# fanzhongyi/ExploreMultiModal

Hardware: AMD Instinct MI355X
Metric: image-text pairs/sec fwd+bwd, VLMo-Base, 1/2/4/8 MI355X; % bf16 MFMA roofline (higher is better)
Workload: dtype bf16

## Files before the change

### exploremultimodal_amd/csrc/attention.hip

```cpp
#include "common.h"
#include "vlmo_hip.h"

namespace {

struct AttnArgs {
    const bf16* qkv;
    const bf16* ctx;
    const bf16* dctx;
    bf16* out;
    float* lse;
    float* qvsum;
    const int32_t* seg;
    const int32_t* keymask;
    int lse_stride, heads, d;
    float scale, scale_log2e;
    uint32_t drop_thresh, drop_cmp;
    float inv_keep;
    uint64_t seed;
    int bh0;
};

#define LOG2E 1.4426950408889634f
#define LN2 0.6931471805599453f

// ... 314 lines not shown
        if (kt + 1 < nq) {
            if (kt + 2 < nq) S0 = s_tile(kt + 2);
            __builtin_amdgcn_sched_barrier(0);
            consume(S1, kt + 1);
            __builtin_amdgcn_sched_barrier(0);
        }
    }
    const float l_run = l2[0] + l2[1];
    const float l_tot = l_run + other_half(l_run);
    if (qi < N) {
        const float inv = a.inv_keep / l_tot;
        bf16* op = a.out + (size_t)qrow * a.d + hd * 64 + 4 * h;
#pragma unroll
        for (int dt = 0; dt < 2; ++dt)
#pragma unroll
            for (int g4 = 0; g4 < 4; ++g4) {
                bf16x4 o = {(bf16)(O[dt][4 * g4 + 0] * inv), (bf16)(O[dt][4 * g4 + 1] * inv),
                            (bf16)(O[dt][4 * g4 + 2] * inv), (bf16)(O[dt][4 * g4 + 3] * inv)};
                *(bf16x4*)(op + dt * 32 + 8 * g4) = o;
            }
        if (h == 0 && a.lse) a.lse[(size_t)bh * a.lse_stride + qi] = (m_run * c2 + log2f(l_tot)) * LN2;
    }
}

__device__ __forceinline__ float half_wave_total(float v) {
    float s_ = v + dpp_mov<0x111, 0xf, 0xf>(v);
    s_ += dpp_mov<0x112, 0xf, 0xf>(v);
    s_ += dpp_mov<0x113, 0xf, 0xf>(v);
    s_ += dpp_mov<0x114, 0xf, 0xe>(s_);
    s_ += dpp_mov<0x118, 0xf, 0xc>(s_);
    s_ += dpp_mov<0x142, 0xa, 0xf>(s_);
    return s_;
}
__device__ __forceinline__ void colsum_tiles(const f32x16* t, float w, float scale, float* acc, int lane) {
    const int h = lane >> 5;
#pragma unroll
    for (int dt = 0; dt < 2; ++dt)
#pragma unroll
        for (int r = 0; r < 16; ++r) {
            const float v = half_wave_total(t[dt][r] * w);
            if ((lane & 31) == 31) atomicAdd(acc + dt * 32 + (r & 3) + 8 * (r >> 2) + 4 * h, v * scale);
        }
}

__global__ __launch_bounds__(512, 2) void attn_bwd_kernel(const AttnArgs a, const int NPAD) {
    const int IMG = NPAD * 128;
    extern __shared__ __attribute__((aligned(16))) char smem[];
    char* Qimg = smem;
    char* Kimg = smem + IMG;
    char* Vimg = smem + 2 * IMG;
    char* Dimg = smem + 3 * IMG;
    float* kbias = (float*)(smem + 4 * IMG);
    float* lseq = kbias + NPAD;
    float* delta = lseq + NPAD;
    int* rowidx = (int*)(delta + NPAD);
    int* next_item = rowidx + NPAD;
    float* csum = (float*)(next_item + 4);

    const int lane = threadIdx.x & 63;
    const int wave = __builtin_amdgcn_readfirstlane(threadIdx.x >> 6);
    const int bh = blockIdx.x, sidx = bh / a.heads, hd = bh % a.heads;
    const int ld = 3 * a.d;
    int N;
    setup_rows(a.seg, sidx, a.keymask, NPAD, rowidx, kbias, N);
    if (threadIdx.x == 0) *next_item = 0;
    if (threadIdx.x < 128) csum[threadIdx.x] = 0.f;
    __syncthreads();
    const int nq = (N + 31) >> 5;
    stage_image<8>(a.qkv, ld, hd * 64, rowidx, Qimg, nq * 4, wave, lane);
    stage_image<8>(a.qkv, ld, a.d + hd * 64, rowidx, Kimg, nq * 4, wave, lane);
    stage_image<8>(a.qkv, ld, 2 * a.d + hd * 64, rowidx, Vimg, nq * 4, wave, lane);
    stage_image<8>(a.dctx, a.d, hd * 64, rowidx, Dimg, nq * 4, wave, lane);
    const float keep_prob = 1.f / a.inv_keep;
    for (int i = threadIdx.x; i < NPAD; i += 512) {
        float dl = 0.f, lq = INFINITY;
        if (i < N) {
            const size_t o = (size_t)rowidx[i] * a.d + hd * 64;
#pragma unroll
            for (int c = 0; c < 8; ++c) {
                const bf16x8 x = *(const bf16x8*)(a.ctx + o + 8 * c);
                const bf16x8 y = *(const bf16x8*)(a.dctx + o + 8 * c);
#pragma unroll
                for (int j = 0; j < 8; ++j) dl += (float)x[j] * (float)y[j];
            }
            lq = a.lse[(size_t)bh * a.lse_stride + i] * LOG2E;
        }
        delta[i] = dl * keep_prob;
        lseq[i] = lq;
    }
    asm volatile("s_waitcnt vmcnt(0)" ::: "memory");
    __syncthreads();

    const int l31 = lane & 31, h = lane >> 5;
    const uint32_t akey = att_key(a.seed, bh + a.bh0);
    const float out_scale = a.scale * a.inv_keep;

    f32x16 cs[2] = {zero16(), zero16()};
    int cs_kind = -1;
    for (;;) {
    int item = 0;
    if (lane == 0) item = atomicAdd(next_item, 1);
    item = __builtin_amdgcn_readfirstlane(item);
    if (a.qvsum) {
        const int kind = item >= 2 * nq ? -1 : (item >= nq ? 0 : 1);
        if (cs_kind >= 0 && kind != cs_kind) {
            colsum_tiles(cs, 1.f, cs_kind == 0 ? out_scale : a.inv_keep, csum + 64 * cs_kind, lane);
            cs[0] = zero16(), cs[1] = zero16();
        }
        cs_kind = kind;
    }
    if (item >= 2 * nq) break;
    if (item >= nq) {
        const int qt = item - nq;
        const int qi = qt * 32 + l31;
        bf16x8 qf[4], df[4];
#pragma unroll
        for (int s = 0; s < 4; ++s) {
            qf[s] = row_frag(Qimg, qt * 32, s, lane);
            df[s] = row_frag(Dimg, qt * 32, s, lane);
        }
        const float lq = lseq[qi], dl = delta[qi];
        const uint32_t rq = ((uint32_t)qi * 512u + 4u * h) * ATT_G + akey;
        f32x16 dQ[2] = {zero16(), zero16()};
        for (int kt = 0; kt < nq; ++kt) {
            {
                f32x16 S = zero16(), dP = zero16();
#pragma unroll
                for (int s = 0; s < 4; ++s) {
                    S = Elem<bf16>::mfma(row_frag(Kimg, kt * 32, s, lane), qf[s], S);
                    dP = Elem<bf16>::mfma(row_frag(Vimg, kt * 32, s, lane), df[s], dP);
                }
                const uint32_t rk = rq + (uint32_t)(kt * 32) * ATT_G;
#pragma unroll
                for (int g4 = 0; g4 < 4; ++g4) {
                    const f32x4 kb = *(const f32x4*)(kbias + kt * 32 + 8 * g4 + 4 * h);
#pragma unroll
                    for (int e = 0; e < 4; ++e) {
                        const int i = 4 * g4 + e;
                        const float p = __builtin_amdgcn_exp2f(S[i] * a.scale_log2e + (kb[e] - lq));
                        bool keep = true;
                        if (a.drop_thresh) keep = att_mix(rk + (uint32_t)(8 * g4 + e) * ATT_G) >= a.drop_cmp;
                        const float dp = keep ? dP[i] : 0.f;
                        S[i] = p * (dp - dl);
                    }
                }
#pragma unroll
                for (int s2 = 0; s2 < 2; ++s2) {
                    bf16x8 sf;
#pragma unroll
                    for (int j = 0; j < 8; ++j) sf[j] = (bf16)S[8 * s2 + j];
#pragma unroll
                    for (int dt = 0; dt < 2; ++dt)
                        dQ[dt] = Elem<bf16>::mfma(tr_frag(Kimg, kt * 32 + 16 * s2, dt * 32, lane), sf, dQ[dt]);
                }
            }
        }
        if (a.qvsum) {
            const float wq = qi < N ? 1.f : 0.f;
#pragma unroll
            for (int dt = 0; dt < 2; ++dt)
#pragma unroll
                for (int r = 0; r < 16; ++r) cs[dt][r] = fmaf(dQ[dt][r], wq, cs[dt][r]);
        }
        if (qi < N) {
            bf16* op = a.out + (size_t)rowidx[qi] * ld + hd * 64 + 4 * h;
#pragma unroll
            for (int dt = 0; dt < 2; ++dt)
#pragma unroll
                for (int g4 = 0; g4 < 4; ++g4) {
                    bf16x4 o = {(bf16)(dQ[dt][4 * g4 + 0] * out_scale), (bf16)(dQ[dt][4 * g4 + 1] * out_scale),
                                (bf16)(dQ[dt][4 * g4 + 2] * out_scale), (bf16)(dQ[dt][4 * g4 + 3] * out_scale)};
                    *(bf16x4*)(op + dt * 32 + 8 * g4) = o;
                }
        }
    }

    else {
        const int kt = item;
        const int ki = kt * 32 + l31;
        bf16x8 kf[4], vf[4];
#pragma unroll
        for (int s = 0; s < 4; ++s) {
            kf[s] = row_frag(Kimg, kt * 32, s, lane);
            vf[s] = row_frag(Vimg, kt * 32, s, lane);
        }
        const float kb = kbias[ki];
        const uint32_t rl = (uint32_t)ki * ATT_G + akey + (uint32_t)(4 * h) * ATT_G512;
        f32x16 dK[2] = {zero16(), zero16()}, dV[2] = {zero16(), zero16()};
        for (int qt = 0; qt < nq; ++qt) {
            {
                f32x16 S = zero16(), dP = zero16();
#pragma unroll
                for (int s = 0; s < 4; ++s) {
                    S = Elem<bf16>::mfma(row_frag(Qimg, qt * 32, s, lane), kf[s], S);
                    dP = Elem<bf16>::mfma(row_frag(Dimg, qt * 32, s, lane), vf[s], dP);
                }
                f32x16 Pd;
                const uint32_t rqt = rl + (uint32_t)(qt * 32) * ATT_G512;
#pragma unroll
                for (int g4 = 0; g4 < 4; ++g4) {
                    const int q0 = qt * 32 + 8 * g4 + 4 * h;
                    const f32x4 lq = *(const f32x4*)(lseq + q0);
                    const f32x4 dl = *(const f32x4*)(delta + q0);
#pragma unroll
                    for (int e = 0; e < 4; ++e) {
                        const int i = 4 * g4 + e;
                        const float p = __builtin_amdgcn_exp2f(S[i] * a.scale_log2e + (kb - lq[e]));
                        bool keep = true;
                        if (a.drop_thresh) keep = att_mix(rqt + (uint32_t)(8 * g4 + e) * ATT_G512) >= a.drop_cmp;
                        Pd[i] = keep ? p : 0.f;
                        S[i] = p * ((keep ? dP[i] : 0.f) - dl[e]);
                    }
                }
#pragma unroll
                for (int s2 = 0; s2 < 2; ++s2) {
                    bf16x8 pf, sf;
#pragma unroll
                    for (int j = 0; j < 8; ++j) {
                        pf[j] = (bf16)Pd[8 * s2 + j];
                        sf[j] = (bf16)S[8 * s2 + j];
                    }
#pragma unroll
                    for (int dt = 0; dt < 2; ++dt) {
                        dV[dt] = Elem<bf16>::mfma(tr_frag(Dimg, qt * 32 + 16 * s2, dt * 32, lane), pf, dV[dt]);
                        dK[dt] = Elem<bf16>::mfma(tr_frag(Qimg, qt * 32 + 16 * s2, dt * 32, lane), sf, dK[dt]);
                    }
                }
            }
        }
        if (a.qvsum) {
            const float wk = ki < N ? 1.f : 0.f;
#pragma unroll
            for (int dt = 0; dt < 2; ++dt)
#pragma unroll
                for (int r = 0; r < 16; ++r) cs[dt][r] = fmaf(dV[dt][r], wk, cs[dt][r]);
        }
        if (ki < N) {
            bf16* op = a.out + (size_t)rowidx[ki] * ld + hd * 64 + 4 * h;
#pragma unroll
            for (int dt = 0; dt < 2; ++dt)
#pragma unroll
                for (int g4 = 0; g4 < 4; ++g4) {
                    bf16x4 ok = {(bf16)(dK[dt][4 * g4 + 0] * out_scale), (bf16)(dK[dt][4 * g4 + 1] * out_scale),
                                 (bf16)(dK[dt][4 * g4 + 2] * out_scale), (bf16)(dK[dt][4 * g4 + 3] * out_scale)};
                    bf16x4 ov = {(bf16)(dV[dt][4 * g4 + 0] * a.inv_keep), (bf16)(dV[dt][4 * g4 + 1] * a.inv_keep),
                                 (bf16)(dV[dt][4 * g4 + 2] * a.inv_keep), (bf16)(dV[dt][4 * g4 + 3] * a.inv_keep)};
                    *(bf16x4*)(op + a.d + dt * 32 + 8 * g4) = ok;
                    *(bf16x4*)(op + 2 * a.d + dt * 32 + 8 * g4) = ov;
                }
        }
    }
    }
    if (a.qvsum) {
        __syncthreads();
        if (threadIdx.x < 128)
            a.qvsum[(size_t)sidx * 2 * a.d + (threadIdx.x >> 6) * a.d + hd * 64 + (threadIdx.x & 63)] = csum[threadIdx.x];
    }
}

__device__ __forceinline__ int slot_off(int k, int q) {
    return k * 64 + ((((q >> 2) ^ (k >> 1)) & 7) << 3) + (q & 3) * 2;
}
__global__ __launch_bounds__(512) void attn_bwd1_kernel(const AttnArgs a, const int NPAD) {
    constexpr bool KF_REG = false;
    const int IMG = NPAD * 128;
    extern __shared__ __attribute__((aligned(16))) char smem[];
    char* Qimg = smem;
    char* Dimg = smem + IMG;
    char* Kimg = smem + 2 * IMG;
    const int nt = NPAD >> 5;
    char* slots = smem + 3 * IMG;
    float* kbias = (float*)(slots + 2 * nt * 2048);
    float* nlq = kbias + NPAD;
    float* ndl = nlq + NPAD;
    float* csum = ndl + NPAD;


    const int lane = threadIdx.x & 63;
    const int w = __builtin_amdgcn_readfirstlane(threadIdx.x >> 6);
    const int nw = blockDim.x >> 6;
    const int bh = blockIdx.x, sidx = bh / a.heads, hd = bh % a.heads;
    const int ld = 3 * a.d;
    const int rowA = a.seg[4 * sidx + 0], lenA = a.seg[4 * sidx + 1], rowB = a.seg[4 * sidx + 2], lenB = a.seg[4 * sidx + 3];
    const int N = lenA + lenB;
    auto rowof = [&](int tok) {
        tok = min(tok, N - 1);
        return tok < lenA ? rowA + tok : rowB + (tok - lenA);
    };
    const int nq = (N + 31) >> 5;
    for (int ii = w; ii < nq * 4; ii += nw) {
        const int chhi = lane >> 5, rowlo = (lane >> 2) & 7, pc = lane & 3;
        const int row = ii * 8 + rowlo;
        const int ch = chhi * 4 + (pc ^ ((row >> 2) & 3));
        const size_t r = (size_t)rowof(row);
        glds16(a.qkv + r * ld + hd * 64 + ch * 8, Qimg + ii * 1024);
        glds16(a.qkv + r * ld + a.d + hd * 64 + ch * 8, Kimg + ii * 1024);
        glds16(a.dctx + r * a.d + hd * 64 + ch * 8, Dimg + ii * 1024);
    }
    const int l31 = lane & 31, h = lane >> 5;
    const bool active = w < nq;
    const int ki = w * 32 + l31;
    const int krow = rowof(ki);
    bf16x8 kf[4], vf[4];
    if (active) {
        const bf16* kp = a.qkv + (size_t)krow * ld + a.d + hd * 64 + 8 * h;
#pragma unroll
        for (int s = 0; s < 4; ++s) {
            if (KF_REG) kf[s] = *(const bf16x8*)(kp + 16 * s);
            vf[s] = *(const bf16x8*)(kp + a.d + 16 * s);
        }
    }
    for (int i = threadIdx.x; i < 128; i += blockDim.x) csum[i] = 0.f;
    const float keep_prob = 1.f / a.inv_keep;
    const float inv_scale = 1.f / a.scale;
    for (int i = threadIdx.x; i < NPAD; i += blockDim.x) {
        float dl = 0.f, lq = INFINITY;
        const int row = rowof(i);
        const bool ok = (i < N) && (!a.keymask || a.keymask[row] != 0);
        if (i < N) {
            const size_t o = (size_t)row * a.d + hd * 64;
            bf16x8 x[8], y[8];
#pragma unroll
            for (int c = 0; c < 8; ++c) {
                x[c] = *(const bf16x8*)(a.ctx + o + 8 * c);
                y[c] = *(const bf16x8*)(a.dctx + o + 8 * c);
            }
            lq = a.lse[(size_t)bh * a.lse_stride + i];
#pragma unroll
            for (int c = 0; c < 8; ++c)
#pragma unroll
                for (int j = 0; j < 8; ++j) dl += (float)x[c][j] * (float)y[c][j];
        }
        kbias[i] = ok ? 0.f : -INFINITY;
        ndl[i] = -dl * keep_prob;
        nlq[i] = -lq * inv_scale;
    }
    asm volatile("s_waitcnt vmcnt(0)" ::: "memory");
    __syncthreads();

    const uint32_t akey = att_key(a.seed, bh + a.bh0);
    const float out_scale = a.scale * a.inv_keep;
    const float c_l2 = a.scale_log2e;
    const float kb = kbias[min(ki, NPAD - 1)];
    const uint32_t rl = (uint32_t)ki * ATT_G + akey + (uint32_t)(4 * h) * ATT_G512;
    f32x16 dK[2] = {zero16(), zero16()}, dV[2] = {zero16(), zero16()}, dQ[2] = {zero16(), zero16()};

    const int xq = (l31 >> 2) & 3;
    const int rf0 = 1024 * (l31 >> 3) + 64 * (l31 & 7) + 16 * (h ^ xq);
    const int rf1 = 1024 * (l31 >> 3) + 64 * (l31 & 7) + 16 * ((2 + h) ^ xq);
    const int tg = (lane >> 4) & 1, tq = (lane >> 2) & 3, tp = lane & 3;
    const int trl = 64 * (4 * h + tq) + 16 * ((2 * tg + (tp >> 1)) ^ h) + 8 * (tp & 1);
    const int trh = 1024 + 64 * (4 * h + tq) + 16 * ((2 * tg + (tp >> 1)) ^ ((2 + h) & 3)) + 8 * (tp & 1);
    auto rfrag = [&](const char* img_rb, int s) -> bf16x8 {
        return *(const bf16x8*)(img_rb + 512 * (s >> 1) + ((s & 1) ? rf1 : rf0));
    };
    auto tfrag = [&](const char* img_rb, int dt) -> bf16x8 {
        const bf16x4 lo = lds_tr4<bf16>(img_rb + 512 * dt + trl);
        const bf16x4 hi = lds_tr4<bf16>(img_rb + 512 * dt + trh);
        return bf16x8{lo[0], lo[1], lo[2], lo[3], hi[0], hi[1], hi[2], hi[3]};
    };
    const int sw0 = slot_off(l31, 4 * h), sw1 = slot_off(l31, 8 + 4 * h);
    const int srl = slot_off(4 * h + tq, 16 * tg + 4 * tp), srh = slot_off(8 + 4 * h + tq, 16 * tg + 4 * tp);
    auto sfrag = [&](const char* slot, int s2) -> bf16x8 {
        const bf16x4 lo = lds_tr4<bf16>(slot + 1024 * s2 + srl);
        const bf16x4 hi = lds_tr4<bf16>(slot + 1024 * s2 + srh);
        return bf16x8{lo[0], lo[1], lo[2], lo[3], hi[0], hi[1], hi[2], hi[3]};
    };

    bf16x8 qa[4], da[4], pf[2], sf[2];
    f32x16 S, dP;
    auto fetch_a = [&](int qt_) {
#pragma unroll
        for (int s = 0; s < 4; ++s) {
            qa[s] = rfrag(Qimg + qt_ * 4096, s);
            da[s] = rfrag(Dimg + qt_ * 4096, s);
        }
    };
    auto qtile = [&](int t_) {
        int q_ = w + t_;
        return q_ >= nq ? q_ - nq : q_;
    };
    auto stage_sdp = [&](int qt) {
        dP = zero16();
#pragma unroll
        for (int g4 = 0; g4 < 4; ++g4) {
            const f32x4 l4 = *(const f32x4*)(nlq + qt * 32 + 8 * g4 + 4 * h);
#pragma unroll
            for (int e = 0; e < 4; ++e) S[4 * g4 + e] = l4[e];
        }
#pragma unroll
        for (int s = 0; s < 4; ++s) {
            const bf16x8 kfs = KF_REG ? kf[s] : rfrag(Kimg + w * 4096, s);
            S = Elem<bf16>::mfma(qa[s], kfs, S);
            dP = Elem<bf16>::mfma(da[s], vf[s], dP);
        }
        __builtin_amdgcn_sched_barrier(0);
    };
    auto stage_valu_dvdk = [&](int qt, int t) {
        bf16x8 dtr[2], qtr[2];
#pragma unroll
        for (int dt = 0; dt < 2; ++dt) {
            dtr[dt] = tfrag(Dimg + qt * 4096, dt);
            qtr[dt] = tfrag(Qimg + qt * 4096, dt);
        }
        __builtin_amdgcn_sched_barrier(0);
        if (a.drop_thresh) {
            const uint32_t rqt = rl + (uint32_t)(qt * 32) * ATT_G512;
#pragma unroll
            for (int g4 = 0; g4 < 4; ++g4) {
                const f32x4 nd = *(const f32x4*)(ndl + qt * 32 + 8 * g4 + 4 * h);
#pragma unroll
                for (int e = 0; e < 4; ++e) {
                    const int i = 4 * g4 + e;
                    const float p = __builtin_amdgcn_exp2f(fmaf(S[i], c_l2, kb));
                    const bool keep = att_mix(rqt + (uint32_t)(8 * g4 + e) * ATT_G512) >= a.drop_cmp;
                    const float pd = keep ? p : 0.f;
                    pf[i >> 3][i & 7] = (bf16)pd;
                    sf[i >> 3][i & 7] = (bf16)fmaf(pd, dP[i], p * nd[e]);
                }
            }
        } else {
#pragma unroll
            for (int g4 = 0; g4 < 4; ++g4) {
                const f32x4 nd = *(const f32x4*)(ndl + qt * 32 + 8 * g4 + 4 * h);
#pragma unroll
                for (int e = 0; e < 4; ++e) {
                    const int i = 4 * g4 + e;
                    const float p = __builtin_amdgcn_exp2f(fmaf(S[i], c_l2, kb));
                    pf[i >> 3][i & 7] = (bf16)p;
                    sf[i >> 3][i & 7] = (bf16)(p * (dP[i] + nd[e]));
                }
            }
        }
        char* myslot = slots + ((t & 1) * nt + w) * 2048;
#pragma unroll
        for (int s2 = 0; s2 < 2; ++s2) {
            *(bf16x4*)(myslot + (sw0 ^ (32 * s2))) = bf16x4{sf[s2][0], sf[s2][1], sf[s2][2], sf[s2][3]};
            *(bf16x4*)(myslot + (sw1 ^ (32 * s2))) = bf16x4{sf[s2][4], sf[s2][5], sf[s2][6], sf[s2][7]};
        }
        __builtin_amdgcn_sched_barrier(0);
        bf16x8 dtr1[2], qtr1[2];
#pragma unroll
        for (int dt = 0; dt < 2; ++dt) {
            dtr1[dt] = tfrag(Dimg + qt * 4096 + 2048, dt);
            qtr1[dt] = tfrag(Qimg + qt * 4096 + 2048, dt);
        }
#pragma unroll
        for (int dt = 0; dt < 2; ++dt) {
            dV[dt] = Elem<bf16>::mfma(dtr[dt], pf[0], dV[dt]);
            dK[dt] = Elem<bf16>::mfma(qtr[dt], sf[0], dK[dt]);
        }
#pragma unroll
        for (int dt = 0; dt < 2; ++dt) {
            dV[dt] = Elem<bf16>::mfma(dtr1[dt], pf[1], dV[dt]);
            dK[dt] = Elem<bf16>::mfma(qtr1[dt], sf[1], dK[dt]);
        }
        __builtin_amdgcn_sched_barrier(0);
    };
    auto stage_dq = [&](int t, int next_q) {
        int wp = w - t;
        if (wp < 0) wp += nq;
        const char* slot = slots + ((t & 1) * nt + wp) * 2048;
        bf16x8 ktr[2][2], sb[2];
#pragma unroll
        for (int s2 = 0; s2 < 2; ++s2) {
            sb[s2] = sfrag(slot, s2);
#pragma unroll
            for (int dt = 0; dt < 2; ++dt) ktr[s2][dt] = tfrag(Kimg + wp * 4096 + 2048 * s2, dt);
        }
        if (next_q >= 0) fetch_a(next_q);
        __builtin_amdgcn_sched_barrier(0);
#pragma unroll
        for (int s2 = 0; s2 < 2; ++s2)
#pragma unroll
            for (int dt = 0; dt < 2; ++dt) dQ[dt] = Elem<bf16>::mfma(ktr[s2][dt], sb[s2], dQ[dt]);
        __builtin_amdgcn_sched_barrier(0);
    };
    if (w >= 4) __builtin_amdgcn_s_setprio(1);
    if (!active) {
        for (int t = 0; t < nq; ++t) __syncthreads();
    } else if (w < 4) {
        fetch_a(w);
        for (int t = 0; t < nq; ++t) {
            const int qt = qtile(t);
            stage_sdp(qt);
            stage_valu_dvdk(qt, t);
            __syncthreads();
            stage_dq(t, t + 1 < nq ? qtile(t + 1) : -1);
        }
    } else {
        fetch_a(w);
        stage_sdp(w);
        for (int t = 0; t < nq; ++t) {
            stage_valu_dvdk(qtile(t), t);
            if (t > 0) stage_dq(t - 1, -1);
            if (t + 1 < nq) {
                fetch_a(qtile(t + 1));
                stage_sdp(qtile(t + 1));
            }
            __syncthreads();
        }
        stage_dq(nq - 1, -1);
    }
    if (active && ki < N) {
        bf16* op = a.out + (size_t)krow * ld + hd * 64 + 4 * h;
#pragma unroll
        for (int dt = 0; dt < 2; ++dt)
#pragma unroll
            for (int g4 = 0; g4 < 4; ++g4) {
                bf16x4 oq = {(bf16)(dQ[dt][4 * g4 + 0] * out_scale), (bf16)(dQ[dt][4 * g4 + 1] * out_scale),
                             (bf16)(dQ[dt][4 * g4 + 2] * out_scale), (bf16)(dQ[dt][4 * g4 + 3] * out_scale)};
                bf16x4 ok = {(bf16)(dK[dt][4 * g4 + 0] * out_scale), (bf16)(dK[dt][4 * g4 + 1] * out_scale),
                             (bf16)(dK[dt][4 * g4 + 2] * out_scale), (bf16)(dK[dt][4 * g4 + 3] * out_scale)};
                bf16x4 ov = {(bf16)(dV[dt][4 * g4 + 0] * a.inv_keep), (bf16)(dV[dt][4 * g4 + 1] * a.inv_keep),
                             (bf16)(dV[dt][4 * g4 + 2] * a.inv_keep), (bf16)(dV[dt][4 * g4 + 3] * a.inv_keep)};
                *(bf16x4*)(op + dt * 32 + 8 * g4) = oq;
                *(bf16x4*)(op + a.d + dt * 32 + 8 * g4) = ok;
                *(bf16x4*)(op + 2 * a.d + dt * 32 + 8 * g4) = ov;
            }
    }
    if (a.qvsum) {
        if (active) {
            const float wt = ki < N ? 1.f : 0.f;
            colsum_tiles(dQ, wt, out_scale, csum, lane);
            colsum_tiles(dV, wt, a.inv_keep, csum + 64, lane);
        }
        __syncthreads();
        for (int i = threadIdx.x; i < 128; i += blockDim.x) {
            float* dst = a.qvsum + (size_t)sidx * 2 * a.d + (i >> 6) * a.d + hd * 64 + (i & 63);
            *dst = csum[i];
        }
    }
}

#define ATT_LW 8
#define ATT_LCH 4
#define ATT_LBUF (ATT_LCH * 4096)
#define ATT_LMAX 1024
#define ATT_LDS_FWD (4 * ATT_LBUF + ATT_LMAX * 4)
#define ATT_LDS_BWD (4 * ATT_LBUF + 3 * ATT_LMAX * 4 + ATT_LW * 64 * 4)

__device__ __forceinline__ uint32_t att_stride(int N) { return N > 512 ? 1024u : 512u; }

struct SeqRows {
    int rowA, lenA, rowB, N;
    __device__ __forceinline__ SeqRows(const int32_t* seg, int sidx)
        : rowA(seg[4 * sidx + 0]), lenA(seg[4 * sidx + 1]), rowB(seg[4 * sidx + 2]), N(seg[4 * sidx + 1] + seg[4 * sidx + 3]) {}
    __device__ __forceinline__ int row(int tok) const {
        tok = min(tok, N - 1);
        return tok < lenA ? rowA + tok : rowB + (tok - lenA);
    }
};

__device__ __forceinline__ void stage_chunk(const bf16* pa, int lda, const bf16* pb, int ldb, const SeqRows& sr, int t0,
                                            int nt, char* ia, char* ib, int w, int lane) {
// ... 748 lines not shown
int& lds_limit_set(int which) {
    static int lim[4][64];
    static bool init = false;
    if (!init) {
        for (auto& r : lim)
            for (int& v : r) v = 65536;
        init = true;
    }
    int dev = 0;
    (void)hipGetDevice(&dev);
    return lim[which][dev & 63];
}

int launch_fwd(const AttnArgs& a, int nt, int nblocks, hipStream_t st) {
    const int LDS = nt * 32 * 256 + nt * 32 * 8;
    int& max_set = lds_limit_set(0);
    if (LDS > max_set) {
        (void)hipFuncSetAttribute((const void*)attn_fwd_kernel, hipFuncAttributeMaxDynamicSharedMemorySize, LDS);
        max_set = LDS;
    }
    hipLaunchKernelGGL(attn_fwd_kernel, dim3(nblocks), dim3(256), LDS, st, a, nt * 32);
    return 0;
}
int launch_fwd1(const AttnArgs& a, int nt, int nblocks, hipStream_t st) {
    const int LDS = nt * 32 * 256 + nt * 32 * 4;
    int& max_set = lds_limit_set(3);
    if (LDS > max_set) {
        (void)hipFuncSetAttribute((const void*)attn_fwd1_kernel, hipFuncAttributeMaxDynamicSharedMemorySize, LDS);
        max_set = LDS;
    }
    hipLaunchKernelGGL(attn_fwd1_kernel, dim3(nblocks), dim3(nt * 64), LDS, st, a, nt * 32);
    return 0;
}
int launch_bwd(const AttnArgs& a, int nt, int nblocks, hipStream_t st) {
    const int LDS = nt * 32 * 512 + nt * 32 * 16 + 32 + 512;
    int& max_set = lds_limit_set(1);
    if (LDS > max_set) {
        (void)hipFuncSetAttribute((const void*)attn_bwd_kernel, hipFuncAttributeMaxDynamicSharedMemorySize, LDS);
        max_set = LDS;
    }
    hipLaunchKernelGGL(attn_bwd_kernel, dim3(nblocks), dim3(512), LDS, st, a, nt * 32);
    return 0;
}

int launch_bwd1(const AttnArgs& a, int nt, int nblocks, hipStream_t st) {
    const int LDS = nt * 32 * 384 + 2 * nt * 2048 + nt * 32 * 12 + 512;
    int& max_set = lds_limit_set(2);
    if (LDS > max_set) {
        (void)hipFuncSetAttribute((const void*)attn_bwd1_kernel, hipFuncAttributeMaxDynamicSharedMemorySize, LDS);
        max_set = LDS;
    }
    hipLaunchKernelGGL(attn_bwd1_kernel, dim3(nblocks), dim3(nt * 64), LDS, st, a, nt * 32);
    return 0;
}

int check_common(const char* fn, const void* qkv, const int32_t* seg, int num_seq, int heads, int d, int max_len,
                 int cap) {
    VLMO_CHECK_ARG(qkv && seg, "%s: null pointer", fn);
    VLMO_CHECK_ARG(num_seq > 0 && heads > 0, "%s: empty problem", fn);
    VLMO_CHECK_ARG(d == heads * 64, "%s: head_dim must be 64 (d=%d, heads=%d)", fn, d, heads);
    VLMO_CHECK_ARG(max_len > 0 && max_len <= cap, "%s: sequence length %d exceeds this build's limit %d", fn, max_len, cap);
    return 0;
}

}

extern "C" int vlmo_attn_fwd(const void* qkv, const int32_t* seg, int num_seq, const int32_t* keymask, void* ctx,
                             float* lse, int lse_stride, int heads, int d, int max_len, float scale,
                             uint32_t drop_thresh, float inv_keep, uint64_t seed, int mask_seq0, hipStream_t stream) {
    if (int rc = check_common("vlmo_attn_fwd", qkv, seg, num_seq, heads, d, max_len, 1024)) return rc;
    VLMO_CHECK_ARG(ctx, "vlmo_attn_fwd: null ctx");
    VLMO_CHECK_ARG(!lse || lse_stride >= max_len, "vlmo_attn_fwd: lse_stride too small");
    AttnArgs a{};
    a.qkv = (const bf16*)qkv;
    a.out = (bf16*)ctx;
    a.lse = lse;
    a.seg = seg;
    a.keymask = keymask;
    a.lse_stride = lse_stride;
    a.heads = heads;
    a.d = d;
    a.scale = scale;
    a.scale_log2e = scale * LOG2E;
    a.drop_thresh = drop_thresh;
    a.drop_cmp = drop_thresh >= 65536u ? 0xFFFFFFFFu : drop_thresh << 16;
// ... 14 lines not shown

extern "C" int vlmo_attn_bwd(const void* qkv, const void* ctx, const void* dctx, const float* lse, int lse_stride,
                             const int32_t* seg, int num_seq, const int32_t* keymask, void* dqkv, float* qv_colsum,
                             int heads, int d, int max_len, float scale, uint32_t drop_thresh, float inv_keep,
                             uint64_t seed, int mask_seq0, hipStream_t stream) {
    if (int rc = check_common("vlmo_attn_bwd", qkv, seg, num_seq, heads, d, max_len, 1024)) return rc;
    VLMO_CHECK_ARG(ctx && dctx && lse && dqkv, "vlmo_attn_bwd: null pointer");
    VLMO_CHECK_ARG(lse_stride >= max_len, "vlmo_attn_bwd: lse_stride too small");
    AttnArgs a{};
    a.qkv = (const bf16*)qkv;
    a.ctx = (const bf16*)ctx;
    a.dctx = (const bf16*)dctx;
    a.out = (bf16*)dqkv;
    a.qvsum = qv_colsum;
    a.lse = (float*)lse;
    a.seg = seg;
    a.keymask = keymask;
    a.lse_stride = lse_stride;
    a.heads = heads;
    a.d = d;
    a.scale = scale;
    a.scale_log2e = scale * LOG2E;
    a.drop_thresh = drop_thresh;
    a.drop_cmp = drop_thresh >= 65536u ? 0xFFFFFFFFu : drop_thresh << 16;
    a.inv_keep = drop_thresh ? inv_keep : 1.f;
    a.seed = seed;
    a.bh0 = mask_seq0 * heads;
    const int nt = (max_len + 31) / 32, nb = num_seq * heads;
    if (max_len > 288) {
        launch_bwd_long(a, nb, stream);
        VLMO_CHECK_LAUNCH("vlmo_attn_bwd(long)");
        return 0;
    }
    if (nt > 8) launch_bwd(a, nt, nb, stream);
    else launch_bwd1(a, nt, nb, stream);
    VLMO_CHECK_LAUNCH("vlmo_attn_bwd");
    return 0;
}

extern "C" int vlmo_attn_probs(const void* qkv, const int32_t* seg, int num_seq, const int32_t* keymask, float* probs,
                               int heads, int d, int seq_len, int q0, int nq, int head_mean, float scale,
                               hipStream_t stream) {
    if (int rc = check_common("vlmo_attn_probs", qkv, seg, num_seq, heads, d, seq_len, ATT_LMAX)) return rc;
    VLMO_CHECK_ARG(probs, "vlmo_attn_probs: null probs");
    VLMO_CHECK_ARG(q0 >= 0 && nq >= 1 && q0 <= seq_len - nq, "vlmo_attn_probs: query rows [%d, %d + %d) outside [0, %d)", q0,
                   q0, nq, seq_len);
    ProbsArgs a{};
    a.qkv = (const bf16*)qkv;
    a.seg = seg;
    a.keymask = keymask;
    a.probs = probs;
    a.heads = heads;
    a.d = d;
    a.seq_len = seq_len;
    a.q0 = q0;
    a.nq = nq;
    a.head_mean = head_mean != 0;
    a.scale_log2e = scale * LOG2E;
    const int gx = num_seq * (a.head_mean ? 1 : heads);
    const int rounds = ((nq + 31) / 32 + ATT_PW - 1) / ATT_PW;
    const int gy = std::min(rounds, std::max(1, (768 + gx - 1) / gx));
    a.tiles_per_block = ATT_PW * ((rounds + gy - 1) / gy);
    launch_probs(a, gx, (rounds * ATT_PW + a.tiles_per_block - 1) / a.tiles_per_block, stream);
    VLMO_CHECK_LAUNCH("vlmo_attn_probs");
    return 0;
}

extern "C" int vlmo_attn_gradcam(const void* qkv, const void* dctx, const int32_t* seg, int num_seq, const int32_t* keymask,
// ... 31 lines not shown
```

Baseline: 4349.

## Replace generic attention backward for 9-tile sequences with fringe-extended pipelined kernel

Removes the atomic work-queue attention backward kernel used when the padded length exceeds 8 tiles. Those cases now go to the 8-wave pipelined bwd1 kernel, templated with a FRINGE path that runs the 8x8 core schedule and then handles the ninth key/query tile. The fringe step stages the extra V tile and computes its dQ with two waves. It merges the partial dK/dV from each wave through LDS reductions. The aim is to bring the faster software-pipelined kernel to lengths up to 288, at the cost of extra serialized fringe work, more syncs and more LDS.

```diff
diff --git a/exploremultimodal_amd/csrc/attention.hip b/exploremultimodal_amd/csrc/attention.hip
--- a/exploremultimodal_amd/csrc/attention.hip
+++ b/exploremultimodal_amd/csrc/attention.hip
@@ -370,235 +370,23 @@
     s_ += dpp_mov<0x142, 0xa, 0xf>(s_);
     return s_;
 }
+__device__ __forceinline__ void colsum_tile(const f32x16& t, float w, float scale, float* acc, int lane) {
+    const int h = lane >> 5;
+#pragma unroll
+    for (int r = 0; r < 16; ++r) {
+        const float v = half_wave_total(t[r] * w);
+        if ((lane & 31) == 31) atomicAdd(acc + (r & 3) + 8 * (r >> 2) + 4 * h, v * scale);
+    }
+}
 __device__ __forceinline__ void colsum_tiles(const f32x16* t, float w, float scale, float* acc, int lane) {
-    const int h = lane >> 5;
-#pragma unroll
-    for (int dt = 0; dt < 2; ++dt)
-#pragma unroll
-        for (int r = 0; r < 16; ++r) {
-            const float v = half_wave_total(t[dt][r] * w);
-            if ((lane & 31) == 31) atomicAdd(acc + dt * 32 + (r & 3) + 8 * (r >> 2) + 4 * h, v * scale);
-        }
-}
-
-__global__ __launch_bounds__(512, 2) void attn_bwd_kernel(const AttnArgs a, const int NPAD) {
-    const int IMG = NPAD * 128;
-    extern __shared__ __attribute__((aligned(16))) char smem[];
-    char* Qimg = smem;
-    char* Kimg = smem + IMG;
-    char* Vimg = smem + 2 * IMG;
-    char* Dimg = smem + 3 * IMG;
-    float* kbias = (float*)(smem + 4 * IMG);
-    float* lseq = kbias + NPAD;
-    float* delta = lseq + NPAD;
-    int* rowidx = (int*)(delta + NPAD);
-    int* next_item = rowidx + NPAD;
-    float* csum = (float*)(next_item + 4);
-
-    const int lane = threadIdx.x & 63;
-    const int wave = __builtin_amdgcn_readfirstlane(threadIdx.x >> 6);
-    const int bh = blockIdx.x, sidx = bh / a.heads, hd = bh % a.heads;
-    const int ld = 3 * a.d;
-    int N;
-    setup_rows(a.seg, sidx, a.keymask, NPAD, rowidx, kbias, N);
-    if (threadIdx.x == 0) *next_item = 0;
-    if (threadIdx.x < 128) csum[threadIdx.x] = 0.f;
-    __syncthreads();
-    const int nq = (N + 31) >> 5;
-    stage_image<8>(a.qkv, ld, hd * 64, rowidx, Qimg, nq * 4, wave, lane);
-    stage_image<8>(a.qkv, ld, a.d + hd * 64, rowidx, Kimg, nq * 4, wave, lane);
-    stage_image<8>(a.qkv, ld, 2 * a.d + hd * 64, rowidx, Vimg, nq * 4, wave, lane);
-    stage_image<8>(a.dctx, a.d, hd * 64, rowidx, Dimg, nq * 4, wave, lane);
-    const float keep_prob = 1.f / a.inv_keep;
-    for (int i = threadIdx.x; i < NPAD; i += 512) {
-        float dl = 0.f, lq = INFINITY;
-        if (i < N) {
-            const size_t o = (size_t)rowidx[i] * a.d + hd * 64;
-#pragma unroll
-            for (int c = 0; c < 8; ++c) {
-                const bf16x8 x = *(const bf16x8*)(a.ctx + o + 8 * c);
-                const bf16x8 y = *(const bf16x8*)(a.dctx + o + 8 * c);
-#pragma unroll
-                for (int j = 0; j < 8; ++j) dl += (float)x[j] * (float)y[j];
-            }
-            lq = a.lse[(size_t)bh * a.lse_stride + i] * LOG2E;
-        }
-        delta[i] = dl * keep_prob;
-        lseq[i] = lq;
-    }
-    asm volatile("s_waitcnt vmcnt(0)" ::: "memory");
-    __syncthreads();
-
-    const int l31 = lane & 31, h = lane >> 5;
-    const uint32_t akey = att_key(a.seed, bh + a.bh0);
-    const float out_scale = a.scale * a.inv_keep;
-
-    f32x16 cs[2] = {zero16(), zero16()};
-    int cs_kind = -1;
-    for (;;) {
-    int item = 0;
-    if (lane == 0) item = atomicAdd(next_item, 1);
-    item = __builtin_amdgcn_readfirstlane(item);
-    if (a.qvsum) {
-        const int kind = item >= 2 * nq ? -1 : (item >= nq ? 0 : 1);
-        if (cs_kind >= 0 && kind != cs_kind) {
-            colsum_tiles(cs, 1.f, cs_kind == 0 ? out_scale : a.inv_keep, csum + 64 * cs_kind, lane);
-            cs[0] = zero16(), cs[1] = zero16();
-        }
-        cs_kind = kind;
-    }
-    if (item >= 2 * nq) break;
-    if (item >= nq) {
-        const int qt = item - nq;
-        const int qi = qt * 32 + l31;
-        bf16x8 qf[4], df[4];
-#pragma unroll
-        for (int s = 0; s < 4; ++s) {
-            qf[s] = row_frag(Qimg, qt * 32, s, lane);
-            df[s] = row_frag(Dimg, qt * 32, s, lane);
-        }
-        const float lq = lseq[qi], dl = delta[qi];
-        const uint32_t rq = ((uint32_t)qi * 512u + 4u * h) * ATT_G + akey;
-        f32x16 dQ[2] = {zero16(), zero16()};
-        for (int kt = 0; kt < nq; ++kt) {
-            {
-                f32x16 S = zero16(), dP = zero16();
-#pragma unroll
-                for (int s = 0; s < 4; ++s) {
-                    S = Elem<bf16>::mfma(row_frag(Kimg, kt * 32, s, lane), qf[s], S);
-                    dP = Elem<bf16>::mfma(row_frag(Vimg, kt * 32, s, lane), df[s], dP);
-                }
-                const uint32_t rk = rq + (uint32_t)(kt * 32) * ATT_G;
-#pragma unroll
-                for (int g4 = 0; g4 < 4; ++g4) {
-                    const f32x4 kb = *(const f32x4*)(kbias + kt * 32 + 8 * g4 + 4 * h);
-#pragma unroll
-                    for (int e = 0; e < 4; ++e) {
-                        const int i = 4 * g4 + e;
-                        const float p = __builtin_amdgcn_exp2f(S[i] * a.scale_log2e + (kb[e] - lq));
-                        bool keep = true;
-                        if (a.drop_thresh) keep = att_mix(rk + (uint32_t)(8 * g4 + e) * ATT_G) >= a.drop_cmp;
-                        const float dp = keep ? dP[i] : 0.f;
-                        S[i] = p * (dp - dl);
-                    }
-                }
-#pragma unroll
-                for (int s2 = 0; s2 < 2; ++s2) {
-                    bf16x8 sf;
-#pragma unroll
-                    for (int j = 0; j < 8; ++j) sf[j] = (bf16)S[8 * s2 + j];
-#pragma unroll
-                    for (int dt = 0; dt < 2; ++dt)
-                        dQ[dt] = Elem<bf16>::mfma(tr_frag(Kimg, kt * 32 + 16 * s2, dt * 32, lane), sf, dQ[dt]);
-                }
-            }
-        }
-        if (a.qvsum) {
-            const float wq = qi < N ? 1.f : 0.f;
-#pragma unroll
-            for (int dt = 0; dt < 2; ++dt)
-#pragma unroll
-                for (int r = 0; r < 16; ++r) cs[dt][r] = fmaf(dQ[dt][r], wq, cs[dt][r]);
-        }
-        if (qi < N) {
-            bf16* op = a.out + (size_t)rowidx[qi] * ld + hd * 64 + 4 * h;
-#pragma unroll
-            for (int dt = 0; dt < 2; ++dt)
-#pragma unroll
-                for (int g4 = 0; g4 < 4; ++g4) {
-                    bf16x4 o = {(bf16)(dQ[dt][4 * g4 + 0] * out_scale), (bf16)(dQ[dt][4 * g4 + 1] * out_scale),
-                                (bf16)(dQ[dt][4 * g4 + 2] * out_scale), (bf16)(dQ[dt][4 * g4 + 3] * out_scale)};
-                    *(bf16x4*)(op + dt * 32 + 8 * g4) = o;
-                }
-        }
-    }
-
-    else {
-        const int kt = item;
-        const int ki = kt * 32 + l31;
-        bf16x8 kf[4], vf[4];
-#pragma unroll
-        for (int s = 0; s < 4; ++s) {
-            kf[s] = row_frag(Kimg, kt * 32, s, lane);
-            vf[s] = row_frag(Vimg, kt * 32, s, lane);
-        }
-        const float kb = kbias[ki];
-        const uint32_t rl = (uint32_t)ki * ATT_G + akey + (uint32_t)(4 * h) * ATT_G512;
-        f32x16 dK[2] = {zero16(), zero16()}, dV[2] = {zero16(), zero16()};
-        for (int qt = 0; qt < nq; ++qt) {
-            {
-                f32x16 S = zero16(), dP = zero16();
-#pragma unroll
-                for (int s = 0; s < 4; ++s) {
-                    S = Elem<bf16>::mfma(row_frag(Qimg, qt * 32, s, lane), kf[s], S);
-                    dP = Elem<bf16>::mfma(row_frag(Dimg, qt * 32, s, lane), vf[s], dP);
-                }
-                f32x16 Pd;
-                const uint32_t rqt = rl + (uint32_t)(qt * 32) * ATT_G512;
-#pragma unroll
-                for (int g4 = 0; g4 < 4; ++g4) {
-                    const int q0 = qt * 32 + 8 * g4 + 4 * h;
-                    const f32x4 lq = *(const f32x4*)(lseq + q0);
-                    const f32x4 dl = *(const f32x4*)(delta + q0);
-#pragma unroll
-                    for (int e = 0; e < 4; ++e) {
-                        const int i = 4 * g4 + e;
-                        const float p = __builtin_amdgcn_exp2f(S[i] * a.scale_log2e + (kb - lq[e]));
-                        bool keep = true;
-                        if (a.drop_thresh) keep = att_mix(rqt + (uint32_t)(8 * g4 + e) * ATT_G512) >= a.drop_cmp;
-                        Pd[i] = keep ? p : 0.f;
-                        S[i] = p * ((keep ? dP[i] : 0.f) - dl[e]);
-                    }
-                }
-#pragma unroll
-                for (int s2 = 0; s2 < 2; ++s2) {
-                    bf16x8 pf, sf;
-#pragma unroll
-                    for (int j = 0; j < 8; ++j) {
-                        pf[j] = (bf16)Pd[8 * s2 + j];
-                        sf[j] = (bf16)S[8 * s2 + j];
-                    }
-#pragma unroll
-                    for (int dt = 0; dt < 2; ++dt) {
-                        dV[dt] = Elem<bf16>::mfma(tr_frag(Dimg, qt * 32 + 16 * s2, dt * 32, lane), pf, dV[dt]);
-                        dK[dt] = Elem<bf16>::mfma(tr_frag(Qimg, qt * 32 + 16 * s2, dt * 32, lane), sf, dK[dt]);
-                    }
-                }
-            }
-        }
-        if (a.qvsum) {
-            const float wk = ki < N ? 1.f : 0.f;
-#pragma unroll
-            for (int dt = 0; dt < 2; ++dt)
-#pragma unroll
-                for (int r = 0; r < 16; ++r) cs[dt][r] = fmaf(dV[dt][r], wk, cs[dt][r]);
-        }
-        if (ki < N) {
-            bf16* op = a.out + (size_t)rowidx[ki] * ld + hd * 64 + 4 * h;
-#pragma unroll
-            for (int dt = 0; dt < 2; ++dt)
-#pragma unroll
-                for (int g4 = 0; g4 < 4; ++g4) {
-                    bf16x4 ok = {(bf16)(dK[dt][4 * g4 + 0] * out_scale), (bf16)(dK[dt][4 * g4 + 1] * out_scale),
-                                 (bf16)(dK[dt][4 * g4 + 2] * out_scale), (bf16)(dK[dt][4 * g4 + 3] * out_scale)};
-                    bf16x4 ov = {(bf16)(dV[dt][4 * g4 + 0] * a.inv_keep), (bf16)(dV[dt][4 * g4 + 1] * a.inv_keep),
-                                 (bf16)(dV[dt][4 * g4 + 2] * a.inv_keep), (bf16)(dV[dt][4 * g4 + 3] * a.inv_keep)};
-                    *(bf16x4*)(op + a.d + dt * 32 + 8 * g4) = ok;
-                    *(bf16x4*)(op + 2 * a.d + dt * 32 + 8 * g4) = ov;
-                }
-        }
-    }
-    }
-    if (a.qvsum) {
-        __syncthreads();
-        if (threadIdx.x < 128)
-            a.qvsum[(size_t)sidx * 2 * a.d + (threadIdx.x >> 6) * a.d + hd * 64 + (threadIdx.x & 63)] = csum[threadIdx.x];
-    }
+#pragma unroll
+    for (int dt = 0; dt < 2; ++dt) colsum_tile(t[dt], w, scale, acc + dt * 32, lane);
 }
 
 __device__ __forceinline__ int slot_off(int k, int q) {
     return k * 64 + ((((q >> 2) ^ (k >> 1)) & 7) << 3) + (q & 3) * 2;
 }
+template <bool FRINGE>
 __global__ __launch_bounds__(512) void attn_bwd1_kernel(const AttnArgs a, const int NPAD) {
     constexpr bool KF_REG = false;
     const int IMG = NPAD * 128;
@@ -612,7 +400,7 @@
     float* nlq = kbias + NPAD;
     float* ndl = nlq + NPAD;
     float* csum = ndl + NPAD;
-
+    char* V8img = (char*)(csum + 128);
 
     const int lane = threadIdx.x & 63;
     const int w = __builtin_amdgcn_readfirstlane(threadIdx.x >> 6);
@@ -621,11 +409,12 @@
     const int ld = 3 * a.d;
     const int rowA = a.seg[4 * sidx + 0], lenA = a.seg[4 * sidx + 1], rowB = a.seg[4 * sidx + 2], lenB = a.seg[4 * sidx + 3];
     const int N = lenA + lenB;
-    auto rowof = [&](int tok) {
+    auto rowof = [&](int tok) __attribute__((always_inline)) {
         tok = min(tok, N - 1);
         return tok < lenA ? rowA + tok : rowB + (tok - lenA);
     };
     const int nq = (N + 31) >> 5;
+    const int nc = FRINGE ? min(nq, 8) : nq;
     for (int ii = w; ii < nq * 4; ii += nw) {
         const int chhi = lane >> 5, rowlo = (lane >> 2) & 7, pc = lane & 3;
         const int row = ii * 8 + rowlo;
@@ -635,8 +424,14 @@
         glds16(a.qkv + r * ld + a.d + hd * 64 + ch * 8, Kimg + ii * 1024);
         glds16(a.dctx + r * a.d + hd * 64 + ch * 8, Dimg + ii * 1024);
     }
+    if (FRINGE && nq > 8 && w >= 4) {
+        const int chhi = lane >> 5, rowlo = (lane >> 2) & 7, pc = lane & 3;
+        const int row = 256 + (w - 4) * 8 + rowlo;
+        const int ch = chhi * 4 + (pc ^ ((row >> 2) & 3));
+        glds16(a.qkv + (size_t)rowof(row) * ld + 2 * a.d + hd * 64 + ch * 8, V8img + (w - 4) * 1024);
+    }
     const int l31 = lane & 31, h = lane >> 5;
-    const bool active = w < nq;
+    const bool active = w < nc;
     const int ki = w * 32 + l31;
     const int krow = rowof(ki);
     bf16x8 kf[4], vf[4];
@@ -679,8 +474,8 @@
     const uint32_t akey = att_key(a.seed, bh + a.bh0);
     const float out_scale = a.scale * a.inv_keep;
     const float c_l2 = a.scale_log2e;
-    const float kb = kbias[min(ki, NPAD - 1)];
-    const uint32_t rl = (uint32_t)ki * ATT_G + akey + (uint32_t)(4 * h) * ATT_G512;
+    const float kb_own = kbias[min(ki, NPAD - 1)];
+    const uint32_t rl_own = (uint32_t)ki * ATT_G + akey + (uint32_t)(4 * h) * ATT_G512;
     f32x16 dK[2] = {zero16(), zero16()}, dV[2] = {zero16(), zero16()}, dQ[2] = {zero16(), zero16()};
 
     const int xq = (l31 >> 2) & 3;
@@ -689,17 +484,17 @@
     const int tg = (lane >> 4) & 1, tq = (lane >> 2) & 3, tp = lane & 3;
     const int trl = 64 * (4 * h + tq) + 16 * ((2 * tg + (tp >> 1)) ^ h) + 8 * (tp & 1);
     const int trh = 1024 + 64 * (4 * h + tq) + 16 * ((2 * tg + (tp >> 1)) ^ ((2 + h) & 3)) + 8 * (tp & 1);
-    auto rfrag = [&](const char* img_rb, int s) -> bf16x8 {
+    auto rfrag = [&](const char* img_rb, int s) __attribute__((always_inline)) -> bf16x8 {
         return *(const bf16x8*)(img_rb + 512 * (s >> 1) + ((s & 1) ? rf1 : rf0));
     };
-    auto tfrag = [&](const char* img_rb, int dt) -> bf16x8 {
+    auto tfrag = [&](const char* img_rb, int dt) __attribute__((always_inline)) -> bf16x8 {
         const bf16x4 lo = lds_tr4<bf16>(img_rb + 512 * dt + trl);
         const bf16x4 hi = lds_tr4<bf16>(img_rb + 512 * dt + trh);
         return bf16x8{lo[0], lo[1], lo[2], lo[3], hi[0], hi[1], hi[2], hi[3]};
     };
     const int sw0 = slot_off(l31, 4 * h), sw1 = slot_off(l31, 8 + 4 * h);
     const int srl = slot_off(4 * h + tq, 16 * tg + 4 * tp), srh = slot_off(8 + 4 * h + tq, 16 * tg + 4 * tp);
-    auto sfrag = [&](const char* slot, int s2) -> bf16x8 {
+    auto sfrag = [&](const char* slot, int s2) __attribute__((always_inline)) -> bf16x8 {
         const bf16x4 lo = lds_tr4<bf16>(slot + 1024 * s2 + srl);
         const bf16x4 hi = lds_tr4<bf16>(slot + 1024 * s2 + srh);
         return bf16x8{lo[0], lo[1], lo[2], lo[3], hi[0], hi[1], hi[2], hi[3]};
@@ -707,18 +502,18 @@
 
     bf16x8 qa[4], da[4], pf[2], sf[2];
     f32x16 S, dP;
-    auto fetch_a = [&](int qt_) {
+    auto fetch_a = [&](int qt_) __attribute__((always_inline)) {
 #pragma unroll
         for (int s = 0; s < 4; ++s) {
             qa[s] = rfrag(Qimg + qt_ * 4096, s);
             da[s] = rfrag(Dimg + qt_ * 4096, s);
         }
     };
-    auto qtile = [&](int t_) {
+    auto qtile = [&](int t_) __attribute__((always_inline)) {
         int q_ = w + t_;
-        return q_ >= nq ? q_ - nq : q_;
+        return q_ >= nc ? q_ - nc : q_;
     };
-    auto stage_sdp = [&](int qt) {
+    auto stage_sdp = [&](int qt, const char* ktile, const bf16x8 (&vfr)[4]) __attribute__((always_inline)) {
         dP = zero16();
 #pragma unroll
         for (int g4 = 0; g4 < 4; ++g4) {
@@ -728,13 +523,14 @@
         }
 #pragma unroll
         for (int s = 0; s < 4; ++s) {
-            const bf16x8 kfs = KF_REG ? kf[s] : rfrag(Kimg + w * 4096, s);
+            const bf16x8 kfs = KF_REG ? kf[s] : rfrag(ktile, s);
             S = Elem<bf16>::mfma(qa[s], kfs, S);
-            dP = Elem<bf16>::mfma(da[s], vf[s], dP);
+            dP = Elem<bf16>::mfma(da[s], vfr[s], dP);
         }
         __builtin_amdgcn_sched_barrier(0);
     };
-    auto stage_valu_dvdk = [&](int qt, int t) {
+    auto stage_valu_dvdk = [&](int qt, char* myslot, float kb, uint32_t rl, f32x16 (&dV)[2],
+                               f32x16 (&dK)[2]) __attribute__((always_inline)) {
         bf16x8 dtr[2], qtr[2];
 #pragma unroll
         for (int dt = 0; dt < 2; ++dt) {
@@ -770,7 +566,6 @@
                 }
             }
         }
-        char* myslot = slots + ((t & 1) * nt + w) * 2048;
 #pragma unroll
         for (int s2 = 0; s2 < 2; ++s2) {
             *(bf16x4*)(myslot + (sw0 ^ (32 * s2))) = bf16x4{sf[s2][0], sf[s2][1], sf[s2][2], sf[s2][3]};
@@ -795,16 +590,13 @@
         }
         __builtin_amdgcn_sched_barrier(0);
     };
-    auto stage_dq = [&](int t, int next_q) {
-        int wp = w - t;
-        if (wp < 0) wp += nq;
-        const char* slot = slots + ((t & 1) * nt + wp) * 2048;
+    auto stage_dq_at = [&](const char* slot, const char* ktile, int next_q) __attribute__((always_inline)) {
         bf16x8 ktr[2][2], sb[2];
 #pragma unroll
         for (int s2 = 0; s2 < 2; ++s2) {
             sb[s2] = sfrag(slot, s2);
 #pragma unroll
-            for (int dt = 0; dt < 2; ++dt) ktr[s2][dt] = tfrag(Kimg + wp * 4096 + 2048 * s2, dt);
+            for (int dt = 0; dt < 2; ++dt) ktr[s2][dt] = tfrag(ktile + 2048 * s2, dt);
         }
         if (next_q >= 0) fetch_a(next_q);
         __builtin_amdgcn_sched_barrier(0);
@@ -814,33 +606,136 @@
             for (int dt = 0; dt < 2; ++dt) dQ[dt] = Elem<bf16>::mfma(ktr[s2][dt], sb[s2], dQ[dt]);
         __builtin_amdgcn_sched_barrier(0);
     };
+    auto stage_dq = [&](int t, int next_q) __attribute__((always_inline)) {
+        int wp = w - t;
+        if (wp < 0) wp += nc;
+        stage_dq_at(slots + ((t & 1) * nt + wp) * 2048, Kimg + wp * 4096, next_q);
+    };
+    const char* kown = Kimg + w * 4096;
+    auto core_sdp = [&](int qt) __attribute__((always_inline)) { stage_sdp(qt, kown, vf); };
+    auto core_valu_dvdk = [&](int qt, int t) __attribute__((always_inline)) {
+        stage_valu_dvdk(qt, slots + ((t & 1) * nt + w) * 2048, kb_own, rl_own, dV, dK);
+    };
     if (w >= 4) __builtin_amdgcn_s_setprio(1);
     if (!active) {
-        for (int t = 0; t < nq; ++t) __syncthreads();
+        for (int t = 0; t < nc; ++t) __syncthreads();
     } else if (w < 4) {
         fetch_a(w);
-        for (int t = 0; t < nq; ++t) {
+        for (int t = 0; t < nc; ++t) {
             const int qt = qtile(t);
-            stage_sdp(qt);
-            stage_valu_dvdk(qt, t);
+            core_sdp(qt);
+            core_valu_dvdk(qt, t);
             __syncthreads();
-            stage_dq(t, t + 1 < nq ? qtile(t + 1) : -1);
+            stage_dq(t, t + 1 < nc ? qtile(t + 1) : -1);
         }
     } else {
         fetch_a(w);
-        stage_sdp(w);
-        for (int t = 0; t < nq; ++t) {
-            stage_valu_dvdk(qtile(t), t);
+        core_sdp(w);
+        for (int t = 0; t < nc; ++t) {
+            core_valu_dvdk(qtile(t), t);
             if (t > 0) stage_dq(t - 1, -1);
-            if (t + 1 < nq) {
+            if (t + 1 < nc) {
                 fetch_a(qtile(t + 1));
-                stage_sdp(qtile(t + 1));
+                core_sdp(qtile(t + 1));
             }
             __syncthreads();
         }
-        stage_dq(nq - 1, -1);
-    }
-    if (active && ki < N) {
+        stage_dq(nc - 1, -1);
+    }
+    if (FRINGE && nq > 8) {
+        auto store_tile = [&](const f32x16 (&t)[2], float sc, int row, int col0) __attribute__((always_inline)) {
+            bf16* op = a.out + (size_t)row * ld + col0 + hd * 64 + 4 * h;
+#pragma unroll
+            for (int dt = 0; dt < 2; ++dt)
+#pragma unroll
+                for (int g4 = 0; g4 < 4; ++g4)
+                    *(bf16x4*)(op + dt * 32 + 8 * g4) =
+                        bf16x4{(bf16)(t[dt][4 * g4 + 0] * sc), (bf16)(t[dt][4 * g4 + 1] * sc),
+                               (bf16)(t[dt][4 * g4 + 2] * sc), (bf16)(t[dt][4 * g4 + 3] * sc)};
+        };
+        fetch_a(8);
+        stage_sdp(8, kown, vf);
+        stage_valu_dvdk(8, slots + w * 2048, kb_own, rl_own, dV, dK);
+        store_tile(dK, out_scale, krow, a.d);
+        store_tile(dV, a.inv_keep, krow, 2 * a.d);
+        if (a.qvsum) colsum_tiles(dV, 1.f, a.inv_keep, csum + 64, lane);
+        dK[0] = zero16(), dK[1] = zero16(), dV[0] = zero16(), dV[1] = zero16();
+        __syncthreads();
+        const int k8 = 256 + l31;
+        const char* k8tile = Kimg + 8 * 4096;
+        const float kb8 = kbias[k8];
+        const uint32_t rl8 = (uint32_t)k8 * ATT_G + akey + (uint32_t)(4 * h) * ATT_G512;
+#pragma unroll
+        for (int s = 0; s < 4; ++s) vf[s] = rfrag(V8img, s);
+        char* slot1 = slots + (nt + w) * 2048;
+        fetch_a(w);
+        stage_sdp(w, k8tile, vf);
+        stage_valu_dvdk(w, slot1, kb8, rl8, dV, dK);
+        stage_dq_at(slot1, k8tile, w == 0 ? 8 : -1);
+        if (w == 0) {
+            stage_sdp(8, k8tile, vf);
+            stage_valu_dvdk(8, slots + 8 * 2048, kb8, rl8, dV, dK);
+        }
+        store_tile(dQ, out_scale, krow, 0);
+        if (a.qvsum) colsum_tiles(dQ, 1.f, out_scale, csum, lane);
+        __syncthreads();
+        auto put = [&](int region) __attribute__((always_inline)) {
+            f32x4* p = (f32x4*)(smem + region * 16384) + lane;
+#pragma unroll
+            for (int dt = 0; dt < 2; ++dt)
+#pragma unroll
+                for (int g4 = 0; g4 < 4; ++g4) {
+                    p[(dt * 4 + g4) * 64] = f32x4{dK[dt][4 * g4], dK[dt][4 * g4 + 1], dK[dt][4 * g4 + 2], dK[dt][4 * g4 + 3]};
+                    p[(8 + dt * 4 + g4) * 64] = f32x4{dV[dt][4 * g4], dV[dt][4 * g4 + 1], dV[dt][4 * g4 + 2], dV[dt][4 * g4 + 3]};
+                }
+        };
+        auto add = [&](int region) __attribute__((always_inline)) {
+            const f32x4* p = (const f32x4*)(smem + region * 16384) + lane;
+#pragma unroll
+            for (int dt = 0; dt < 2; ++dt)
+#pragma unroll
+                for (int g4 = 0; g4 < 4; ++g4) {
+                    const f32x4 uk = p[(dt * 4 + g4) * 64], uv = p[(8 + dt * 4 + g4) * 64];
+#pragma unroll
+                    for (int e = 0; e < 4; ++e) dK[dt][4 * g4 + e] += uk[e], dV[dt][4 * g4 + e] += uv[e];
+                }
+        };
+        const int row8 = rowof(k8);
+        const float wt8 = k8 < N ? 1.f : 0.f;
+        if (w >= 4) put(w - 4);
+        if (w == 4 || w == 5) {
+            const int dt = w - 4;
+            f32x16 acc = zero16();
+            for (int k = 0; k < 9; ++k) {
+                const char* slot = slots + k * 2048;
+                const bf16x8 s0 = sfrag(slot, 0), s1 = sfrag(slot, 1);
+                const bf16x8 k0 = tfrag(Kimg + k * 4096, dt), k1 = tfrag(Kimg + k * 4096 + 2048, dt);
+                acc = Elem<bf16>::mfma(k0, s0, acc);
+                acc = Elem<bf16>::mfma(k1, s1, acc);
+            }
+            if (k8 < N) {
+                bf16* op = a.out + (size_t)row8 * ld + hd * 64 + dt * 32 + 4 * h;
+#pragma unroll
+                for (int g4 = 0; g4 < 4; ++g4)
+                    *(bf16x4*)(op + 8 * g4) =
+                        bf16x4{(bf16)(acc[4 * g4 + 0] * out_scale), (bf16)(acc[4 * g4 + 1] * out_scale),
+                               (bf16)(acc[4 * g4 + 2] * out_scale), (bf16)(acc[4 * g4 + 3] * out_scale)};
+            }
+            if (a.qvsum) colsum_tile(acc, wt8, out_scale, csum + dt * 32, lane);
+        }
+        __syncthreads();
+        if (w < 4) add(w);
+        if (w >= 1 && w < 4) put(w);
+        __syncthreads();
+        if (w == 0) {
+            add(1), add(2), add(3);
+            if (k8 < N) {
+                store_tile(dK, out_scale, row8, a.d);
+                store_tile(dV, a.inv_keep, row8, 2 * a.d);
+            }
+            if (a.qvsum) colsum_tiles(dV, wt8, a.inv_keep, csum + 64, lane);
+        }
+    } else if (active && ki < N) {
         bf16* op = a.out + (size_t)krow * ld + hd * 64 + 4 * h;
 #pragma unroll
         for (int dt = 0; dt < 2; ++dt)
@@ -858,7 +753,7 @@
             }
     }
     if (a.qvsum) {
-        if (active) {
+        if (active && !(FRINGE && nq > 8)) {
             const float wt = ki < N ? 1.f : 0.f;
             colsum_tiles(dQ, wt, out_scale, csum, lane);
             colsum_tiles(dV, wt, a.inv_keep, csum + 64, lane);
@@ -1673,25 +1568,16 @@
     hipLaunchKernelGGL(attn_fwd1_kernel, dim3(nblocks), dim3(nt * 64), LDS, st, a, nt * 32);
     return 0;
 }
-int launch_bwd(const AttnArgs& a, int nt, int nblocks, hipStream_t st) {
-    const int LDS = nt * 32 * 512 + nt * 32 * 16 + 32 + 512;
-    int& max_set = lds_limit_set(1);
+template <bool FRINGE>
+int launch_bwd1(const AttnArgs& a, int nt, int nblocks, hipStream_t st) {
+    const int LDS = nt * 32 * 384 + 2 * nt * 2048 + nt * 32 * 12 + 512 + (FRINGE ? 4096 : 0);
+    if (LDS > 160 * 1024) return -1;
+    int& max_set = lds_limit_set(FRINGE ? 1 : 2);
     if (LDS > max_set) {
-        (void)hipFuncSetAttribute((const void*)attn_bwd_kernel, hipFuncAttributeMaxDynamicSharedMemorySize, LDS);
+        (void)hipFuncSetAttribute((const void*)attn_bwd1_kernel<FRINGE>, hipFuncAttributeMaxDynamicSharedMemorySize, LDS);
         max_set = LDS;
     }
-    hipLaunchKernelGGL(attn_bwd_kernel, dim3(nblocks), dim3(512), LDS, st, a, nt * 32);
-    return 0;
-}
-
-int launch_bwd1(const AttnArgs& a, int nt, int nblocks, hipStream_t st) {
-    const int LDS = nt * 32 * 384 + 2 * nt * 2048 + nt * 32 * 12 + 512;
-    int& max_set = lds_limit_set(2);
-    if (LDS > max_set) {
-        (void)hipFuncSetAttribute((const void*)attn_bwd1_kernel, hipFuncAttributeMaxDynamicSharedMemorySize, LDS);
-        max_set = LDS;
-    }
-    hipLaunchKernelGGL(attn_bwd1_kernel, dim3(nblocks), dim3(nt * 64), LDS, st, a, nt * 32);
+    hipLaunchKernelGGL(attn_bwd1_kernel<FRINGE>, dim3(nblocks), dim3((FRINGE ? 8 : nt) * 64), LDS, st, a, nt * 32);
     return 0;
 }
 
@@ -1772,8 +1658,8 @@
         VLMO_CHECK_LAUNCH("vlmo_attn_bwd(long)");
         return 0;
     }
-    if (nt > 8) launch_bwd(a, nt, nb, stream);
-    else launch_bwd1(a, nt, nb, stream);
+    const int rc = nt > 8 ? launch_bwd1<true>(a, nt, nb, stream) : launch_bwd1<false>(a, nt, nb, stream);
+    VLMO_CHECK_ARG(rc == 0, "vlmo_attn_bwd: %d tokens do not fit the LDS of one CU", max_len);
     VLMO_CHECK_LAUNCH("vlmo_attn_bwd");
     return 0;
 }
```

Result: faster. 4397, median of 6 (+1.1%).
